# mouzzarr/go-libp2p-pubsub

Hardware: AMD Instinct MI355X
Metric: peer-heartbeat updates/sec + msg-edge deliveries/sec, 1M-peer gossipsub sim (higher is better)
Workload: dtype f64; 1 GPU; c3: 1000000 peers, random-regular k=32, one IP per peer, 16 topics, beacon-style params, 4 msg/s/topic, 10 rounds/heartbeat; peers_per_gpu=1000000, degree=32, topics=16, edge_topic_records=512000000, rounds_per_heartbeat=10

## Files before the change

### go-libp2p-pubsub_amd/csrc/deliver.hip

```cpp
#include <algorithm>
#include <cstdlib>
#include <vector>

#include "gsim_internal.h"
#include "philox.h"

namespace gsim {

#ifndef GSIM_IH_MASK
#define GSIM_IH_MASK 1
#endif
constexpr int kIhMaskSlots = 128;
__device__ __forceinline__ bool bit128(uint64_t w0, uint64_t w1, int k)
{
    return ((k < 64 ? w0 >> k : w1 >> (k - 64)) & 1ull) != 0;
}

constexpr int64_t kMaxPromTicks = 64;
constexpr int kMaxRing = 8192;

__device__ __forceinline__ bool verdict_penalises(uint8_t v)
{
    return v == GSIM_VERDICT_REJECT || v == GSIM_VERDICT_SIGNATURE;
}
// ... 1618 lines not shown
}

template <bool LAT, bool SP>
__global__ __launch_bounds__(256) void k_gossip_count(IhArgs a, uint32_t* gcount)
{
    extern __shared__ uint16_t s_act[];
    __shared__ int s_n;
    uint32_t* s_cnt = reinterpret_cast<uint32_t*>(s_act + ((a.ring + 1) & ~1));
    for (int w = threadIdx.x; w < 2 * a.ring; w += blockDim.x) s_cnt[w] = 0;
    if (threadIdx.x < 64) {
        const int lane = threadIdx.x;
        int n = 0;
        for (int m0 = 0; m0 < a.ring; m0 += 64) {
            const int m = m0 + lane;
            const bool act = m < a.ring && a.slot_last[m] >= a.lo_round;
            const uint64_t b = __ballot(act);
            if (act) s_act[n + __popcll(b & ((1ull << lane) - 1))] = (uint16_t)m;
            n += __popcll(b);
        }
        if (lane == 0) s_n = n;
    }
    __syncthreads();
    if (blockIdx.x == 0 && threadIdx.x == 0 && s_n > a.max_ihave) atomicOr(&a.nresp[3], 4u);
    const int lane = threadIdx.x & 63;
    const int64_t p0 = ((int64_t)blockIdx.x * 4 + (threadIdx.x >> 6)) * 64;
    const int nact = p0 < a.CN ? s_n : 0;
    const int64_t pc = p0 + lane, pl = pc;
    const bool vp = pc < a.CN;
    const uint64_t subp = vp ? a.sub[pl] : 0ull;
    const int64_t tick_round = a.tick * a.R;
    for (int k0 = 0; k0 < nact; k0 += kSlotBatch) {
        uint64_t cv[kSlotBatch];
#pragma unroll
        for (int b = 0; b < kSlotBatch; ++b) {
            const int k = k0 + b;
            const int64_t ci = (k < nact && vp) ? word_cell<SP>(a.cs, a.mtopic, s_act[k], p0 >> 6, lane) : -1;
            cv[b] = ci >= 0 ? a.cs.cell[ci] : kUnseen64;
        }
#pragma unroll
        for (int b = 0; b < kSlotBatch; ++b) {
            const int k = k0 + b;
            if (k >= nact) break;
            const uint32_t m = s_act[k];
            const int32_t t = (int32_t)a.mtopic[m];
            const bool hold = vp && holds_in_window(cv[b], a.g, a.lo_round, tick_round, a.minv[m] != 0,
                                                   (uint32_t)pl == a.morigin[m], LAT ? a.mlat[m] : 0u);
            const bool want = vp && cv[b] == kUnseen64 && ((subp >> t) & 1ull) && pl >= a.rlo && pl < a.rhi;
            const int nh = __popcll(__ballot(hold)), nw = __popcll(__ballot(want));
            if (lane == 0 && nh) atomicAdd(&s_cnt[m], (uint32_t)nh);
            if (lane == 0 && nw) atomicAdd(&s_cnt[a.ring + m], (uint32_t)nw);
        }
    }
    __syncthreads();
    for (int w = threadIdx.x; w < 2 * a.ring; w += blockDim.x)
        if (s_cnt[w]) atomicAdd(&gcount[w], s_cnt[w]);
}

#ifndef GSIM_COUNT_BATCH
#define GSIM_COUNT_BATCH 4
#endif
constexpr int kCountBatch = GSIM_COUNT_BATCH;
template <bool LAT>
__global__ __launch_bounds__(256) void k_gossip_count_mm(IhArgs a, const uint32_t* mctab, uint32_t* gcount)
{
    extern __shared__ uint32_t s_c[];
    __shared__ uint16_t s_slot[kMaxRing / 8];
    __shared__ int s_n;
    const int32_t t = block_topic(mctab, a.T, blockIdx.x);
    const int32_t R = a.topic_slots, m_lo = t * R;
    for (int w = threadIdx.x; w < 2 * R; w += blockDim.x) s_c[w] = 0;
    const int lane = threadIdx.x & 63, wid = threadIdx.x >> 6;
    if (threadIdx.x < 64) {
        int n = 0;
        for (int k0 = 0; k0 < R; k0 += 64) {
            const int k = k0 + lane;
            const bool act = k < R && a.slot_last[m_lo + k] >= a.lo_round;
            const uint64_t b = __ballot(act);
            if (act) s_slot[n + __popcll(b & ((1ull << lane) - 1))] = (uint16_t)k;
            n += __popcll(b);
        }
        if (lane == 0) s_n = n;
    }
    __syncthreads();
    if (blockIdx.x == 0 && threadIdx.x < 64) {
        int tot = 0;
        for (int m0 = 0; m0 < a.ring; m0 += 64)
            tot += __popcll(__ballot(m0 + lane < a.ring && a.slot_last[m0 + lane] >= a.lo_round));
        if (lane == 0 && tot > a.max_ihave) atomicOr(&a.nresp[3], 4u);
    }
    const int ns = s_n;
    const int64_t M = a.mcount[t];
    const int64_t tick_round = a.tick * a.R;
    for (int64_t j0 = (int64_t)(blockIdx.x - mctab[t]) * 1024 + wid * 64; j0 < M && ns; j0 += 256) {
        if (j0 >= (int64_t)(blockIdx.x - mctab[t] + 1) * 1024) break;
        const int64_t j = j0 + lane;
        const bool vp = j < M;
        const uint32_t p = vp ? member_peer(a, t, j) : 0u;
        const bool subp = vp && ((a.sub[p] >> t) & 1ull) && p >= a.rlo && p < a.rhi;
        uint64_t hw0 = 0, hw1 = 0, uw0 = 0, uw1 = 0;
        for (int q0 = 0; q0 < ns; q0 += kCountBatch) {
          uint64_t cb[kCountBatch];
#pragma unroll
          for (int b = 0; b < kCountBatch; ++b)
              cb[b] = (vp && q0 + b < ns) ? a.cs.cell[(int64_t)a.cs.cbase[m_lo + s_slot[q0 + b]] + j] : kUnseen64;
#pragma unroll
          for (int b = 0; b < kCountBatch; ++b) {
            const int q = q0 + b;
            if (q >= ns) break;
            const int k = s_slot[q];
            const uint32_t m = (uint32_t)(m_lo + k);
            const uint64_t c = cb[b];
            const bool hold = vp && holds_in_window(c, a.g, a.lo_round, tick_round, a.minv[m] != 0, p == a.morigin[m],
                                                    LAT ? a.mlat[m] : 0u);
            const bool want = subp && c == kUnseen64;
            const uint64_t kb = 1ull << (k & 63);
            if (hold) { if (k < 64) hw0 |= kb; else hw1 |= kb; }
            if (c == kUnseen64) { if (k < 64) uw0 |= kb; else uw1 |= kb; }
            const int nh = __popcll(__ballot(hold)), nw = __popcll(__ballot(want));
            if (lane == 0 && nh) atomicAdd(&s_c[k], (uint32_t)nh);
            if (lane == 0 && nw) atomicAdd(&s_c[R + k], (uint32_t)nw);
          }
        }
        if (a.ihm && vp) {
            uint64_t* o = a.ihm + (a.mmb[t] + j) * 4;
            o[0] = hw0; o[1] = hw1; o[2] = uw0; o[3] = uw1;
        }
    }
    __syncthreads();
    for (int w = threadIdx.x; w < 2 * R; w += blockDim.x)
        if (s_c[w]) atomicAdd(&gcount[(w < R ? 0 : a.ring - R) + m_lo + w], s_c[w]);
}

#ifndef GSIM_IH_WPE
#define GSIM_IH_WPE 4
#endif
#ifndef GSIM_IH_BATCH
#define GSIM_IH_BATCH 4
#endif
constexpr int kIhBatch = GSIM_IH_BATCH;
#ifndef GSIM_IH_HUB
#define GSIM_IH_HUB 1024
#endif
#ifndef GSIM_IH_SLICES
#define GSIM_IH_SLICES 8
#endif
constexpr uint32_t kIhHub = GSIM_IH_HUB;
constexpr int kIhSlices = GSIM_IH_SLICES;
#ifdef GSIM_DIAG_IH
__device__ unsigned long long g_ih_diag[16];
#define IH_D(...) __VA_ARGS__
#else
#define IH_D(...)
#endif
template <int W, bool LAT, bool SP, bool MM = false, int LP = 0>
__global__ __launch_bounds__(256, MM ? GSIM_IH_WPE : 1) void k_ihave(IhArgs a_, const uint32_t* gcount)
{
    const IhArgs& a = a_;
    extern __shared__ uint16_t s_act[];
    __shared__ int s_n;
    if (a.nresp[3] & 4u) return;
    const int wid = threadIdx.x >> 6;
    uint64_t* stage = reinterpret_cast<uint64_t*>(s_act + ((a.ring + 3) & ~3)) + wid * kRespStage;
    const uint32_t hw = LP == 2 ? a.hubw[blockIdx.x / kIhSlices] : 0u;
    const uint32_t bx = LP == 2 ? (hw & 0x07FFFFFFu) >> 2 : blockIdx.x;
    const int wsel = LP == 2 ? (int)(hw & 3u) : wid;
    const uint32_t slice = LP == 2 ? blockIdx.x % kIhSlices : 0u;
    const uint32_t nsl = LP == 2 ? (hw >> 27) + 1u : 1u;
    if (LP == 2 && slice >= nsl) return;
    const int32_t tb = MM ? block_topic(a.mmtab, a.T, bx) : 0;
    const int64_t jb = MM ? (int64_t)(bx - a.mmtab[tb]) * 256 : 0;
    const int m_lo = MM ? tb * a.topic_slots : 0, m_hi = MM ? m_lo + a.topic_slots : a.ring;
    if (threadIdx.x < 64) {
        const int lane = threadIdx.x;
        int n = 0;
        for (int m0 = m_lo; m0 < m_hi; m0 += 64) {
            const int m = m0 + lane;
            const bool act = m < m_hi && a.slot_last[m] >= a.lo_round && gcount[m] != 0 && gcount[a.ring + m] != 0;
            const bool push = act && (uint64_t)gcount[m] * 4u < (uint64_t)gcount[a.ring + m] * 32u;
            const uint64_t b = __ballot(act);
            if (act) s_act[n + __popcll(b & ((1ull << lane) - 1))] = (uint16_t)(m | (push ? 0x8000 : 0));
            n += __popcll(b);
        }
        if (lane == 0) s_n = n;
    }
    __syncthreads();
    const int lane = threadIdx.x & 63;
    const int64_t p0 = MM ? 0 : ((int64_t)blockIdx.x * 4 + wid) * 64;
    const int64_t jw = jb + wsel * 64;
    const int nact = (MM ? jw < a.mcount[tb] : p0 < a.CN) ? s_n : 0;
    const bool vp = MM ? jw + lane < a.mcount[tb] : p0 + lane < a.CN;
    const int64_t pl = MM ? (vp ? (int64_t)member_peer(a, tb, jw + lane) : 0) : p0 + lane;
    const int grp = lane / W, gl = lane % W;
    const uint64_t gmask = group_mask<W>(grp);
    const uint64_t subp = vp ? a.sub[pl] : 0ull;
    const uint32_t rp0 = vp ? a.row_ptr[pl] : 0u;
    const uint32_t rp1 = vp ? a.row_ptr[pl + 1] : 0u;
    const bool ign_l = vp && (a.behaviour[pl] & GSIM_BEHAVE_IGNORE_IWANT);
    const uint64_t long_lanes = W < 64 ? __ballot(rp1 - rp0 > 4u * (uint32_t)W) : 0ull;
    const uint64_t hub_lanes = LP ? __ballot(rp1 - rp0 > kIhHub) : 0ull;
    bool had_hub = false;
    uint32_t hub_max = LP == 1 && rp1 - rp0 > kIhHub ? rp1 - rp0 : 0u;
    if constexpr (LP == 1)
        for (int o = 32; o; o >>= 1) hub_max = max(hub_max, (uint32_t)__shfl_xor((int)hub_max, o, 64));
    const int64_t tick_round = a.tick * a.R;
    int nstage = 0;
    unsigned long long n_walk = 0, n_req = 0, n_resp = 0;
    auto flush_stage = [&]() {
        __builtin_amdgcn_wave_barrier();
        __builtin_amdgcn_fence(__ATOMIC_ACQ_REL, "wavefront");
        uint32_t base = 0;
        if (lane == 0 && nstage) base = atomicAdd(&a.nresp[0], (uint32_t)nstage);
        base = __shfl(base, 0, 64);
        for (int q = lane; q < nstage; q += 64) {
            if ((int64_t)base + q < a.resp_cap) a.resp[base + q] = stage[q];
            else atomicOr(&a.nresp[1], 1u);
        }
        nstage = 0;
    };
    for (int k0 = 0; !MM && k0 < nact; k0 += kSlotBatch) {
        uint64_t cv[kSlotBatch];
#pragma unroll
        for (int b = 0; b < kSlotBatch; ++b) {
            const int k = k0 + b;
            const int64_t ci = (k < nact && vp)
                                   ? (MM ? (int64_t)a.cs.cbase[s_act[k] & 0x7FFF] + jw + lane
                                         : word_cell<SP>(a.cs, a.mtopic, s_act[k] & 0x7FFF, p0 >> 6, lane))
                                   : -1;
            cv[b] = ci >= 0 ? a.cs.cell[ci] : kUnseen64;
        }
#pragma unroll
        for (int b = 0; b < kSlotBatch; ++b) {
            const IhArgs& a = kernarg0(a_);
            const int k = k0 + b;
            if (k >= nact) break;
            const uint32_t m = s_act[k] & 0x7FFF;
            const bool push = (s_act[k] & 0x8000) != 0;
            const int32_t t = (int32_t)a.mtopic[m];
            const uint32_t origin = a.morigin[m];
            const bool inv = a.minv[m] != 0;
            const bool me = vp && (push ? holds_in_window(cv[b], a.g, a.lo_round, tick_round, inv, (uint32_t)pl == origin,
                                                          LAT ? a.mlat[m] : 0u)
                                        : (cv[b] == kUnseen64 && ((subp >> t) & 1ull) && pl >= a.rlo && pl < a.rhi));
            const uint64_t mask = __ballot(me);
            if (!mask) continue;
            const int64_t cb_m = (int64_t)a.cs.cbase[m];
            auto chunk = [&](uint32_t off, uint32_t gl_, uint32_t beg, uint32_t deg, uint32_t me_id, uint32_t me_g,
                             bool ign_s, int64_t me_pl) {
                const bool v = off + gl_ < deg;
                const uint32_t e = beg + off + gl_;
                bool req = false, resp = false;
                uint32_t r = 0;
                if (push) {
                    if (v && me_pl >= 0 && a.gsel[me_pl + e]) {
                        const uint32_t p = a.col[e], re = a.rev[e];
                        const int64_t pci = a.cs.at(cb_m, t, p);
                        req = p >= a.rlo && p < a.rhi && a.gstate[re] && pci >= 0 && a.cs.cell[pci] == kUnseen64;
                        if (req) {
                            if (a.tr.ev) trace_iwant(a, p, me_id, m);
                            const uint64_t key = pair_key(a.seed, (uint32_t)a.tick, a.gid ? a.gid[p] : p, 0, P_PROMISE,
                                                          m, me_g);
                            atomicMin(reinterpret_cast<unsigned long long*>(&a.pcand[re]), (unsigned long long)key);
                            r = e;
                            resp = a.respond && a.gstate[e] && !ign_s && peertx_allows(a, m, e, me_id);
                        }
                    }
                } else {
                    if (v) {
                        const uint32_t re = a.rev[e];
                        const uint32_t i = a.col[e];
                        const uint64_t mi = smask_of(a.smask, i);
                        if (slot_has(mi, t) && a.gsel[slot_idx(mi, t, a.E, re)] && a.gstate[e]) {
                            const int64_t ici = a.cs.at(cb_m, t, i);
                            req = holds_in_window(ici >= 0 ? a.cs.cell[ici] : kUnseen64, a.g, a.lo_round, tick_round, inv,
                                                  i == origin, LAT ? a.mlat[m] : 0u);
                            if (req) {
                                if (a.tr.ev) trace_iwant(a, me_id, i, m);
                                const uint64_t key = pair_key(a.seed, (uint32_t)a.tick, me_g, 0, P_PROMISE, m,
                                                              a.gid ? a.gid[i] : i);
                                atomicMin(reinterpret_cast<unsigned long long*>(&a.pcand[e]), (unsigned long long)key);
                                r = re;
                                resp = a.respond && a.gstate[re] && !(a.behaviour[i] & GSIM_BEHAVE_IGNORE_IWANT) &&
                                       peertx_allows(a, m, re, i);
                            }
                        }
                    }
                }
                n_req += req;
                n_resp += resp;
                const uint64_t sb = __ballot(resp);
                if (sb) {
                    if (nstage + __popcll(sb) > kRespStage) flush_stage();
                    if (resp) stage[nstage + __popcll(sb & ((1ull << lane) - 1))] = (uint64_t)r | ((uint64_t)m << 32);
                    nstage += __popcll(sb);
                }
            };
            const uint64_t longm = mask & long_lanes;
            uint64_t gm = mask & ~longm & gmask;
            while (__ballot(gm != 0)) {
                int bs = -1;
                if (gm) { bs = __ffsll((long long)gm) - 1; gm &= gm - 1; }
                const int sl = bs < 0 ? lane : bs;
                const uint32_t beg = __shfl(rp0, sl, 64), end = __shfl(rp1, sl, 64);
                const bool ign_s = __shfl(ign_l, sl, 64);
                const uint32_t me_id = MM ? (uint32_t)__shfl((int)pl, sl, 64) : (uint32_t)(p0 + (bs < 0 ? 0 : bs));
                const uint32_t me_g = a.gid ? a.gid[me_id] : me_id;
                const uint64_t me_m = smask_of(a.smask, me_id);
                const int64_t me_pl = slot_has(me_m, t) ? slot_idx(me_m, t, a.E, 0) : -1;
                n_walk += (gl == 0 && bs >= 0);
                const uint32_t deg = bs >= 0 ? end - beg : 0u;
                for (uint32_t off = 0; __ballot(off < deg) != 0; off += W)
                    chunk(off, (uint32_t)gl, beg, deg, me_id, me_g, ign_s, me_pl);
            }
            for (uint64_t lm = longm; lm; lm &= lm - 1) {
                const int bs = __builtin_ctzll(lm);
                const uint32_t beg = __shfl(rp0, bs, 64), end = __shfl(rp1, bs, 64);
                const bool ign_s = __shfl(ign_l, bs, 64);
                const uint32_t me_id = MM ? (uint32_t)__shfl((int)pl, bs, 64) : (uint32_t)(p0 + bs);
                const uint32_t me_g = a.gid ? a.gid[me_id] : me_id;
                const uint64_t me_m = smask_of(a.smask, me_id);
                const int64_t me_pl = slot_has(me_m, t) ? slot_idx(me_m, t, a.E, 0) : -1;
                n_walk += (lane == 0);
                for (uint32_t off = 0; off < end - beg; off += 64)
                    chunk(off, (uint32_t)lane, beg, end - beg, me_id, me_g, ign_s, me_pl);
            }
        }
    }
    IH_D(unsigned long long d_pw = 0, d_pe = 0, d_ph = 0, d_qw = 0, d_qe = 0, d_qh = 0, d_pc = 0, d_qc = 0;)
    if constexpr (MM) {
        IH_D(const unsigned long long c_p0 = clock64();)
        const bool msk = a.ihm != nullptr;
        uint64_t ih0 = 0, ih1 = 0, iu0 = 0, iu1 = 0;
        if (msk && vp) {
            const uint64_t* o = a.ihm + (a.mmb[tb] + jw + lane) * 4;
            ih0 = o[0]; ih1 = o[1]; iu0 = o[2]; iu1 = o[3];
        }
        int64_t own_pl = -1;
        if (vp) {
            const uint64_t om = smask_of(a.smask, (uint32_t)pl);
            own_pl = slot_has(om, tb) ? slot_idx(om, tb, a.E, 0) : -1;
        }
        uint64_t pk0 = 0, pk1 = 0;
        if (msk) {
            for (int q = lane; q < nact; q += 64) {
                const uint16_t sa = s_act[q];
                if (!(sa & 0x8000)) continue;
                const int k = (int)(sa & 0x7FFF) - m_lo;
                if (k < 64) pk0 |= 1ull << k; else pk1 |= 1ull << (k - 64);
            }
            for (int o = 32; o; o >>= 1) {
                pk0 |= (uint64_t)__shfl_xor((long long)pk0, o, 64);
                pk1 |= (uint64_t)__shfl_xor((long long)pk1, o, 64);
            }
        }
        for (int k0 = 0; k0 < nact; k0 += msk ? nact : 64) {
            const int kn = nact - k0 < 64 ? nact - k0 : 64;
            uint64_t hm = 0, hm1 = 0;
            if (msk) {
                if (vp) { hm = ih0 & pk0; hm1 = ih1 & pk1; }
            } else {
                for (int q = 0; q < kn; ++q) {
                    const uint16_t sa = s_act[k0 + q];
                    if (!(sa & 0x8000)) continue;
                    const uint32_t m = sa & 0x7FFF;
                    const uint64_t c = vp ? a.cs.cell[(int64_t)a.cs.cbase[m] + jw + lane] : kUnseen64;
                    if (vp && holds_in_window(c, a.g, a.lo_round, tick_round, a.minv[m] != 0, (uint32_t)pl == a.morigin[m],
                                              LAT ? a.mlat[m] : 0u))
                        hm |= 1ull << q;
                }
            }
            const uint64_t mask = __ballot((hm | hm1) != 0);
            if (!mask) continue;
            const int32_t t = tb;
            auto ask_one = [&](bool req, uint32_t m, uint32_t p, uint32_t pg, uint32_t re, uint32_t e, uint32_t me_id,
                               uint32_t me_g, bool ign_s) {
                bool resp = false;
                if (req) {
                    if (a.tr.ev) trace_iwant(a, p, me_id, m);
                    const uint64_t key = pair_key(a.seed, (uint32_t)a.tick, pg, 0, P_PROMISE, m, me_g);
                    atomicMin(reinterpret_cast<unsigned long long*>(&a.pcand[re]), (unsigned long long)key);
                    resp = a.respond && a.gstate[e] && !ign_s && peertx_allows(a, m, e, me_id);
                }
                n_req += req;
                n_resp += resp;
                const uint64_t sb = __ballot(resp);
                if (sb) {
                    if (nstage + __popcll(sb) > kRespStage) flush_stage();
                    if (resp) stage[nstage + __popcll(sb & ((1ull << lane) - 1))] = (uint64_t)e | ((uint64_t)m << 32);
                    nstage += __popcll(sb);
                }
            };
            auto hchunk = [&](uint32_t off, uint32_t gl_, uint32_t beg, uint32_t deg, uint32_t me_id, uint32_t me_g,
                              bool ign_s, int64_t me_pl, uint64_t hmw, uint64_t hmw1) {
                const bool v = off + gl_ < deg;
                const uint32_t e = beg + off + gl_;
                uint32_t p = 0, re = 0;
                bool gs = false;
                if (v && me_pl >= 0 && a.gsel[me_pl + e]) {
                    p = a.col[e];
                    re = a.rev[e];
                    gs = p >= a.rlo && p < a.rhi && a.gstate[re];
                    IH_D(d_ph++;)
                }
                IH_D(d_pe += v;)
                const uint32_t pg = gs ? (a.gid ? a.gid[p] : p) : 0u;
                const int64_t poff = gs ? a.cs.at(0, t, p) : -1;
                if (msk) {
                    uint64_t r0 = 0, r1 = 0;
                    if (poff >= 0) {
                        const uint64_t* o = a.ihm + (a.mmb[t] + poff) * 4 + 2;
                        r0 = hmw & o[0];
                        r1 = hmw1 & o[1];
                    }
                    while (__ballot((r0 | r1) != 0)) {
                        int k = -1;
                        if (r0) { k = __builtin_ctzll(r0); r0 &= r0 - 1; }
                        else if (r1) { k = 64 + __builtin_ctzll(r1); r1 &= r1 - 1; }
                        ask_one(k >= 0, (uint32_t)(m_lo + (k < 0 ? 0 : k)), p, pg, re, e, me_id, me_g, ign_s);
                    }
                    return;
                }
                const uint64_t mine = gs ? hmw : 0ull;
                uint64_t uw = mine;
                for (int o = 32; o; o >>= 1) uw |= (uint64_t)__shfl_xor((long long)uw, o, 64);
                while (uw) {
                  int qb[kIhBatch];
                  bool ask[kIhBatch];
                  uint64_t cvb[kIhBatch];
#pragma unroll
                  for (int b = 0; b < kIhBatch; ++b) {
                      qb[b] = uw ? __builtin_ctzll(uw) : -1;
                      if (uw) uw &= uw - 1;
                      ask[b] = qb[b] >= 0 && ((mine >> qb[b]) & 1ull) && poff >= 0;
                      cvb[b] = ask[b] ? a.cs.cell[(int64_t)a.cs.cbase[s_act[k0 + qb[b]] & 0x7FFF] + poff] : 0ull;
                  }
#pragma unroll
                  for (int b = 0; b < kIhBatch; ++b) {
                    const int q = qb[b];
                    if (q < 0) break;
                    ask_one(ask[b] && cvb[b] == kUnseen64, s_act[k0 + q] & 0x7FFF, p, pg, re, e, me_id, me_g, ign_s);
                  }
                }
            };
            had_hub = had_hub || (mask & hub_lanes) != 0;
            const uint64_t longm = LP == 2 ? (mask & hub_lanes) : LP == 1 ? (mask & long_lanes & ~hub_lanes)
                                                                           : (mask & long_lanes);
            uint64_t gm = LP == 2 ? 0ull : (mask & ~long_lanes & gmask);
            while (__ballot(gm != 0)) {
                int bs = -1;
                if (gm) { bs = __ffsll((long long)gm) - 1; gm &= gm - 1; }
                const int sl = bs < 0 ? lane : bs;
                const uint32_t beg = __shfl(rp0, sl, 64), end = __shfl(rp1, sl, 64);
                const bool ign_s = __shfl(ign_l, sl, 64);
                const uint32_t me_id = (uint32_t)__shfl((int)pl, sl, 64);
                const uint64_t hmw = bs < 0 ? 0ull : (uint64_t)__shfl((long long)hm, sl, 64);
                const uint64_t hmw1 = bs < 0 ? 0ull : (uint64_t)__shfl((long long)hm1, sl, 64);
                const uint32_t me_g = a.gid ? a.gid[me_id] : me_id;
                const int64_t me_pl = (int64_t)__shfl((long long)own_pl, sl, 64);
                n_walk += (gl == 0 && bs >= 0);
                IH_D(d_pw += (gl == 0 && bs >= 0);)
                const uint32_t deg = bs >= 0 ? end - beg : 0u;
                for (uint32_t off = 0; __ballot(off < deg) != 0; off += W)
                    hchunk(off, (uint32_t)gl, beg, deg, me_id, me_g, ign_s, me_pl, hmw, hmw1);
            }
            for (uint64_t lm = longm; lm; lm &= lm - 1) {
                const int bs = __builtin_ctzll(lm);
                const uint32_t beg = __shfl(rp0, bs, 64), end = __shfl(rp1, bs, 64);
                const bool ign_s = __shfl(ign_l, bs, 64);
                const uint32_t me_id = (uint32_t)__shfl((int)pl, bs, 64);
                const uint64_t hmw = (uint64_t)__shfl((long long)hm, bs, 64);
                const uint64_t hmw1 = (uint64_t)__shfl((long long)hm1, bs, 64);
                const uint32_t me_g = a.gid ? a.gid[me_id] : me_id;
                const int64_t me_pl = (int64_t)__shfl((long long)own_pl, bs, 64);
                n_walk += (lane == 0 && slice == 0);
                IH_D(d_pw += (lane == 0 && slice == 0);)
                for (uint32_t off = slice * 64; off < end - beg; off += 64 * nsl)
                    hchunk(off, (uint32_t)lane, beg, end - beg, me_id, me_g, ign_s, me_pl, hmw, hmw1);
            }
        }
        IH_D(const unsigned long long c_p1 = clock64(); d_pc += c_p1 - c_p0;)
        const bool rcv = vp && ((subp >> tb) & 1ull) && pl >= a.rlo && pl < a.rhi;
        for (int k0 = 0; k0 < nact; k0 += 64) {
            const int kn = nact - k0 < 64 ? nact - k0 : 64;
            uint64_t wm = 0;
            for (int q = 0; q < kn; ++q) {
                const uint16_t sa = s_act[k0 + q];
                if (sa & 0x8000) continue;
                if (msk) {
                    if (rcv && bit128(iu0, iu1, (int)(sa & 0x7FFF) - m_lo)) wm |= 1ull << q;
                    continue;
                }
                const uint64_t c = rcv ? a.cs.cell[(int64_t)a.cs.cbase[sa & 0x7FFF] + jw + lane] : 0ull;
                if (rcv && c == kUnseen64) wm |= 1ull << q;
            }
            const uint64_t mask = __ballot(wm != 0);
            if (!mask) continue;
            const int32_t t = tb;
            auto pchunk = [&](uint32_t off, uint32_t gl_, uint32_t beg, uint32_t deg, uint32_t me_id, uint32_t me_g, uint64_t wmw) {
                const bool v = off + gl_ < deg;
                const uint32_t e = beg + off + gl_;
                uint32_t re = 0, i = 0;
                bool gs = false;
                if (v) {
                    re = a.rev[e];
                    i = a.col[e];
                    const uint64_t mi = smask_of(a.smask, i);
                    gs = slot_has(mi, t) && a.gsel[slot_idx(mi, t, a.E, re)] && a.gstate[e];
                }
                IH_D(d_qe += v; d_qh += gs;)
                const uint64_t mine = gs ? wmw : 0ull;
                uint64_t uw = mine;
                for (int o = 32; o; o >>= 1) uw |= (uint64_t)__shfl_xor((long long)uw, o, 64);
                const uint32_t ig = gs ? (a.gid ? a.gid[i] : i) : 0u;
                const int64_t ioff = gs ? a.cs.at(0, t, i) : -1;
                uint64_t ah0 = 0, ah1 = 0;
                if (msk && ioff >= 0) {
                    const uint64_t* o = a.ihm + (a.mmb[t] + ioff) * 4;
                    ah0 = o[0]; ah1 = o[1];
                }
                while (uw) {
                  int qb[kIhBatch];
                  uint64_t cvb[kIhBatch];
#pragma unroll
                  for (int b = 0; b < kIhBatch; ++b) {
                      qb[b] = uw ? __builtin_ctzll(uw) : -1;
                      if (uw) uw &= uw - 1;
                      const bool ask = qb[b] >= 0 && ((mine >> qb[b]) & 1ull) && ioff >= 0;
                      const uint32_t mb = ask ? s_act[k0 + qb[b]] & 0x7FFF : 0u;
                      cvb[b] = !ask ? kUnseen64 : msk ? (bit128(ah0, ah1, (int)mb - m_lo) ? 1ull : kUnseen64)
                                                      : a.cs.cell[(int64_t)a.cs.cbase[mb] + ioff];
                  }
#pragma unroll
                  for (int b = 0; b < kIhBatch; ++b) {
                    const int q = qb[b];
                    if (q < 0) break;
                    const uint32_t m = s_act[k0 + q] & 0x7FFF;
                    bool req = false, resp = false;
                    if ((mine >> q) & 1ull) {
                        req = msk ? cvb[b] != kUnseen64
                                  : holds_in_window(cvb[b], a.g, a.lo_round, tick_round,
                                                    a.minv[m] != 0, i == a.morigin[m], LAT ? a.mlat[m] : 0u);
                        if (req) {
                            if (a.tr.ev) trace_iwant(a, me_id, i, m);
                            const uint64_t key = pair_key(a.seed, (uint32_t)a.tick, me_g, 0, P_PROMISE, m, ig);
                            atomicMin(reinterpret_cast<unsigned long long*>(&a.pcand[e]), (unsigned long long)key);
                            resp = a.respond && a.gstate[re] && !(a.behaviour[i] & GSIM_BEHAVE_IGNORE_IWANT) &&
                                   peertx_allows(a, m, re, i);
                        }
                    }
                    n_req += req;
                    n_resp += resp;
                    const uint64_t sb = __ballot(resp);
                    if (sb) {
                        if (nstage + __popcll(sb) > kRespStage) flush_stage();
                        if (resp) stage[nstage + __popcll(sb & ((1ull << lane) - 1))] = (uint64_t)re | ((uint64_t)m << 32);
                        nstage += __popcll(sb);
                    }
                  }
                }
            };
            had_hub = had_hub || (mask & hub_lanes) != 0;
            const uint64_t longm = LP == 2 ? (mask & hub_lanes) : LP == 1 ? (mask & long_lanes & ~hub_lanes)
                                                                           : (mask & long_lanes);
            uint64_t gm = LP == 2 ? 0ull : (mask & ~long_lanes & gmask);
            while (__ballot(gm != 0)) {
                int bs = -1;
                if (gm) { bs = __ffsll((long long)gm) - 1; gm &= gm - 1; }
                const int sl = bs < 0 ? lane : bs;
                const uint32_t beg = __shfl(rp0, sl, 64), end = __shfl(rp1, sl, 64);
                const uint32_t me_id = (uint32_t)__shfl((int)pl, sl, 64);
                const uint64_t wmw = bs < 0 ? 0ull : (uint64_t)__shfl((long long)wm, sl, 64);
                const uint32_t me_g = a.gid ? a.gid[me_id] : me_id;
                n_walk += (gl == 0 && bs >= 0);
                IH_D(d_qw += (gl == 0 && bs >= 0);)
                const uint32_t deg = bs >= 0 ? end - beg : 0u;
                for (uint32_t off = 0; __ballot(off < deg) != 0; off += W) pchunk(off, (uint32_t)gl, beg, deg, me_id, me_g, wmw);
            }
            for (uint64_t lm = longm; lm; lm &= lm - 1) {
                const int bs = __builtin_ctzll(lm);
                const uint32_t beg = __shfl(rp0, bs, 64), end = __shfl(rp1, bs, 64);
                const uint32_t me_id = (uint32_t)__shfl((int)pl, bs, 64);
                const uint64_t wmw = (uint64_t)__shfl((long long)wm, bs, 64);
                const uint32_t me_g = a.gid ? a.gid[me_id] : me_id;
                n_walk += (lane == 0 && slice == 0);
                IH_D(d_qw += (lane == 0 && slice == 0);)
                for (uint32_t off = slice * 64; off < end - beg; off += 64 * nsl)
                    pchunk(off, (uint32_t)lane, beg, end - beg, me_id, me_g, wmw);
            }
        }
        IH_D(d_qc += clock64() - c_p1;)
        if constexpr (LP == 1) {
            if (had_hub && lane == 0) {
                const uint32_t ns = (uint32_t)kIhSlices;
                (void)hub_max;
                a.hubw[atomicAdd(a.hubn, 1u)] = (blockIdx.x * 4u + (uint32_t)wid) | ((ns - 1u) << 27);
            }
        }
    }
    flush_stage();
#ifdef GSIM_DIAG_IH
    if (MM && LP) {
        unsigned long long* dg = g_ih_diag + (LP == 2 ? 8 : 0);
        const unsigned long long v6[6] = {wave_sum_u64(d_pw), wave_sum_u64(d_pe), wave_sum_u64(d_ph),
                                          wave_sum_u64(d_qw), wave_sum_u64(d_qe), wave_sum_u64(d_qh)};
        if (lane == 0) {
            for (int q = 0; q < 6; ++q) if (v6[q]) atomicAdd(&dg[q], v6[q]);
            atomicAdd(&dg[6], d_pc);
            atomicAdd(&dg[7], d_qc);
        }
    }
#endif
    n_walk = wave_sum_u64(n_walk);
    n_req = wave_sum_u64(n_req);
    n_resp = wave_sum_u64(n_resp);
    if (lane == 0 && (n_walk | n_req)) {
        atomicAdd(&a.gstats[0], n_walk);
        atomicAdd(&a.gstats[1], n_req);
        atomicAdd(&a.gstats[2], n_resp);
    }
}

constexpr int kPairTopics = 64;

template <bool LAT>
__global__ __launch_bounds__(256) void k_ihave_pairs(IhArgs a)
{
    extern __shared__ uint16_t s_act[];
    __shared__ int s_n;
    if (!(a.nresp[3] & 4u)) return;
    const int wid = threadIdx.x >> 6, lane = threadIdx.x & 63;
    uint64_t* base = reinterpret_cast<uint64_t*>(s_act + ((a.ring + 3) & ~3));
    uint64_t* stage = base + wid * kRespStage;
    uint64_t* s_tau = base + 4 * kRespStage + wid * kPairTopics;
    uint32_t* s_cnt = reinterpret_cast<uint32_t*>(base + 4 * kRespStage + 4 * kPairTopics) + wid * kPairTopics;
    if (threadIdx.x < 64) {
        int n = 0;
        for (int m0 = 0; m0 < a.ring; m0 += 64) {
            const int m = m0 + lane;
            const bool act = m < a.ring && a.slot_last[m] >= a.lo_round;
            const uint64_t b = __ballot(act);
            if (act) s_act[n + __popcll(b & ((1ull << lane) - 1))] = (uint16_t)m;
            n += __popcll(b);
        }
        if (lane == 0) s_n = n;
    }
    __syncthreads();
    const int ns = s_n;
    const uint32_t L = (uint32_t)a.max_ihave;
    const int64_t tick_round = a.tick * a.R;
    int nstage = 0;
    unsigned long long n_walk = 0, n_req = 0, n_resp = 0;
    auto flush_stage = [&]() {
        __builtin_amdgcn_wave_barrier();
        __builtin_amdgcn_fence(__ATOMIC_ACQ_REL, "wavefront");
        uint32_t b0 = 0;
        if (lane == 0 && nstage) b0 = atomicAdd(&a.nresp[0], (uint32_t)nstage);
        b0 = __shfl(b0, 0, 64);
        for (int q = lane; q < nstage; q += 64) {
            if ((int64_t)b0 + q < a.resp_cap) a.resp[b0 + q] = stage[q];
            else atomicOr(&a.nresp[1], 1u);
        }
        nstage = 0;
    };
    auto lds_sync = [&]() {
        __builtin_amdgcn_fence(__ATOMIC_RELEASE, "wavefront");
        __builtin_amdgcn_wave_barrier();
        __builtin_amdgcn_fence(__ATOMIC_ACQUIRE, "wavefront");
    };
    auto kth_key = [&](auto sel) -> uint64_t {
        uint64_t lo = 0, hi = ~0ull;
        while (lo < hi) {
            const uint64_t mid = lo + ((hi - lo) >> 1);
            uint32_t c = 0;
            for (int k0 = 0; k0 < ns; k0 += 64) {
                const int k = k0 + lane;
                uint64_t key = 0;
                c += (uint32_t)__popcll(__ballot(k < ns && sel(k, key) && key <= mid));
            }
            if (c >= L) hi = mid; else lo = mid + 1;
        }
        return lo;
    };
    for (int64_t pc = (int64_t)blockIdx.x * 4 + wid; pc < a.CN; pc += (int64_t)gridDim.x * 4) {
        const uint32_t p = (uint32_t)pc;
        if (p < a.rlo || p >= a.rhi) continue;
        const uint64_t subp = a.sub[p];
        const uint32_t beg = a.row_ptr[p], end = a.row_ptr[p + 1];
        const uint32_t p_g = a.gid ? a.gid[p] : p;
        for (uint32_t e = beg; e < end; ++e) {
            if (!a.gstate[e]) continue;
            const uint32_t re = a.rev[e], i = a.col[e];
            const uint64_t mi = smask_of(a.smask, i);
            const bool tb = lane < a.T && ((subp >> lane) & 1ull) && slot_has(mi, lane) &&
                            a.gsel[slot_idx(mi, lane, a.E, re)];
            const uint64_t tmask = __ballot(tb);
            if (!tmask) continue;
            n_walk += (lane == 0);
            const uint32_t i_g = a.gid ? a.gid[i] : i;
            const uint32_t origin_ign = a.behaviour[i] & GSIM_BEHAVE_IGNORE_IWANT;
            auto holds = [&](uint32_t m) {
                return holds_in_window(a.cs.get(m, (int32_t)a.mtopic[m], i), a.g, a.lo_round, tick_round, a.minv[m] != 0,
                                       i == a.morigin[m], LAT ? a.mlat[m] : 0u);
            };
            s_cnt[lane] = 0;
            lds_sync();
            for (int k0 = 0; k0 < ns; k0 += 64) {
                const int k = k0 + lane;
                if (k < ns) {
                    const uint32_t m = s_act[k];
                    const int t = (int)a.mtopic[m];
                    if (((tmask >> t) & 1ull) && holds(m)) atomicAdd(&s_cnt[t], 1u);
                }
            }
            lds_sync();
            const uint64_t omask = __ballot(s_cnt[lane] > L) & tmask;
            for (uint64_t om = omask; om; om &= om - 1) {
                const int t = __ffsll((long long)om) - 1;
                const uint64_t tau = kth_key([&](int k, uint64_t& key) {
                    const uint32_t m = s_act[k];
                    if ((int)a.mtopic[m] != t || !holds(m)) return false;
                    key = pair_key(a.seed, (uint32_t)a.tick, i_g, (uint32_t)t, P_IHAVE_TRUNC, m, p_g);
                    return true;
                });
                if (lane == 0) s_tau[t] = tau;
            }
            lds_sync();
            auto wanted = [&](uint32_t m) {
                const int t = (int)a.mtopic[m];
                if (!((tmask >> t) & 1ull) || a.cs.get(m, t, p) != kUnseen64 || !holds(m)) return false;
                return s_cnt[t] <= L ||
                       pair_key(a.seed, (uint32_t)a.tick, i_g, (uint32_t)t, P_IHAVE_TRUNC, m, p_g) <= s_tau[t];
            };
            uint32_t nw = 0;
            for (int k0 = 0; k0 < ns; k0 += 64) {
                const int k = k0 + lane;
                nw += (uint32_t)__popcll(__ballot(k < ns && wanted(s_act[k])));
            }
            if (nw == 0) continue;
            uint64_t tau_w = ~0ull;
            if (nw > L)
                tau_w = kth_key([&](int k, uint64_t& key) {
                    const uint32_t m = s_act[k];
                    if (!wanted(m)) return false;
                    key = pair_key(a.seed, (uint32_t)a.tick, p_g, 0, P_IWANT, m, i_g);
                    return true;
                });
            uint64_t pmin = ~0ull;
            for (int k0 = 0; k0 < ns; k0 += 64) {
                const int k = k0 + lane;
                const uint32_t m = k < ns ? s_act[k] : 0u;
                const bool ask = k < ns && wanted(m) &&
                                 (nw <= L || pair_key(a.seed, (uint32_t)a.tick, p_g, 0, P_IWANT, m, i_g) <= tau_w);
                bool resp = false;
                if (ask) {
// ... 783 lines not shown
int deliver_promise_check(gsim_handle* h, int64_t now)
{
    Deliver* d = h->dl;
    if (!d) return GSIM_OK;
    for (int q = 0; q < d->prom_ticks; ++q) {
        const int64_t made = d->prom_made[(size_t)q];
        if (made < 0) continue;
        const int64_t expire = round_time_host(d, made * d->cfg.rounds) + h->gp.iwant_followup_time_ns;
        if (!(expire < now)) continue;
        hipLaunchKernelGGL(k_promise_check, dim3(std::min<int64_t>((h->e + 255) / 256, 16384)), dim3(256), 0,
                           h->stream, d->d_prom + (size_t)q * (size_t)h->e, deliver_cells(d),
                           (const uint32_t*)d->d_mtopic, (const uint32_t*)h->d_owner, (const uint32_t*)h->d_rev,
                           h->d_pen, h->e, d->d_gstats);
        d->prom_made[(size_t)q] = -1;
        int rc = hip_check(h, hipGetLastError(), "k_promise_check");
        if (rc) return rc;
    }
    return GSIM_OK;
}

int deliver_heartbeat_begin(gsim_handle* h, uint64_t tick)
{
    Deliver* d = h->dl;
    if (!d) return GSIM_OK;
    d->ihave_tick = (int64_t)tick;
    return GSIM_OK;
}

namespace gsim {
struct IhaveStage {
    IhArgs a{};
    size_t lds, lds_c;
    int grid;
};
}

static bool ihave_prepare(gsim_handle* h, int64_t g, IhaveStage* st, int* rc)
{
    *rc = GSIM_OK;
    Deliver* d = h->dl;
    const int64_t tick = g / d->cfg.rounds;
    if (d->ihave_tick != tick) return false;
    d->ihave_tick = -1;
    if (h->gp.max_ihave_messages < 1 || h->gp.max_ihave_length < 1) return false;
    IhArgs& a = st->a;
    a = IhArgs{};
    a.N = h->n; a.E = h->e; a.T = h->t; a.ring = d->cfg.ring; a.R = d->cfg.rounds;
    a.g = g; a.tick = tick;
    a.lo_round = (int32_t)std::max<int64_t>((tick - h->gp.history_gossip) * d->cfg.rounds, 0);
    a.serve_lo = (int32_t)std::max<int64_t>((tick - h->gp.history_length + 1) * d->cfg.rounds, 0);
    a.row_ptr = h->d_row_ptr; a.col = h->d_col; a.rev = h->d_rev; a.sub = h->d_sub; a.smask = h->d_smask;
    a.mtopic = d->d_mtopic; a.morigin = d->d_morigin; a.minv = d->d_minv;
    a.mlat = d->lat_on ? d->d_mlat : nullptr;
    a.cs = deliver_cells(d); a.slot_last = d->d_slot_last;
    a.gsel = d->d_gsel; a.gstate = d->d_gstate; a.behaviour = d->d_behaviour;
    a.pcand = d->d_pcand; a.prom = d->d_prom; a.P = d->prom_ticks;
    a.prom_idx = (int32_t)(tick % d->prom_ticks);
    if (d->prom_made[(size_t)a.prom_idx] >= 0) {
        h->err = "IWANT promise ring index still pending (refresh_scores must run every heartbeat)";
        *rc = GSIM_ESTATE;
        return false;
    }
    d->prom_made[(size_t)a.prom_idx] = tick;
    a.resp = d->d_resp; a.nresp = d->d_nresp; a.resp_cap = d->resp_cap; a.gstats = d->d_gstats;
    a.respond = h->gp.gossip_retransmission >= 1;
    a.seed = h->x ? gsim_get_seed(h) : 0;
    a.CN = h->n;
    a.rlo = (uint32_t)h->olo();
    a.rhi = (uint32_t)h->ohi();
    if (ShardCtx* sh = h->sh) {
        a.sharded = 1;
        a.gid = sh->d_gid;
    }
    a.max_ihave = h->gp.max_ihave_length;
    a.tr = h->trace;
    a.t0 = d->cfg.t0_ns; a.hb = d->cfg.heartbeat_ns; a.roff = d->d_roff;
    a.peertx = d->d_peertx; a.ptx_w = d->ptx_w;
    a.retrans = h->gp.gossip_retransmission;
    if (mm_gossip(h)) {
        a.mlist = d->d_mlist; a.mloff = d->d_mloff; a.mcount = d->d_mcount; a.mmtab = d->d_mmtab;
        a.topic_slots = (int32_t)d->cfg.topic_slots;
        a.ihm = d->d_ihm; a.mmb = d->d_mmb;
        const int64_t need = 4 * (int64_t)(d->mmtab.empty() ? 0 : d->mmtab.back());
        if (need > d->hubw_cap) {
            if (d->d_hubw) { (void)hipFree(d->d_hubw); d->d_hubw = nullptr; d->hubw_cap = 0; }
            if (hipMalloc((void**)&d->d_hubw, sizeof(uint32_t) * (size_t)(need + 1)) == hipSuccess) d->hubw_cap = need;
        }
        if (d->d_hubw && need > 0) {
            a.hubw = d->d_hubw;
            a.hubn = d->d_hubw + d->hubw_cap;
        }
    }
    st->lds = (((size_t)d->cfg.ring + 3) & ~(size_t)3) * sizeof(uint16_t) + 4 * kRespStage * sizeof(uint64_t);
    st->lds_c = (((size_t)d->cfg.ring + 1) & ~(size_t)1) * sizeof(uint16_t) + 2 * (size_t)d->cfg.ring * 4;
    st->grid = grid_peers(a.CN);
    hipError_t e = hipMemsetAsync(d->d_nresp, 0, 2 * sizeof(uint32_t), h->stream);
    if (e == hipSuccess) e = hipMemsetAsync(d->d_nresp + 3, 0, sizeof(uint32_t), h->stream);
    if (e == hipSuccess) e = hipMemsetAsync(d->d_gcount, 0, 2 * (size_t)d->cfg.ring * 4, h->stream);
    if (e != hipSuccess) { *rc = hip_check(h, e, "gossip reset"); return false; }
    return true;
}

static int ihave_count(gsim_handle* h, IhaveStage* st)
{
    ProfScope ps(h, GSIM_K_GOSSIP);
    Deliver* d = h->dl;
    if (st->a.mmtab) {
        const uint32_t grid = d->mctab.back();
        const size_t lds = 2 * (size_t)d->cfg.topic_slots * 4;
        if (grid && st->a.mlat)
            hipLaunchKernelGGL(k_gossip_count_mm<true>, dim3(grid), dim3(256), lds, h->stream, st->a,
                               (const uint32_t*)d->d_mctab, d->d_gcount);
        else if (grid)
            hipLaunchKernelGGL(k_gossip_count_mm<false>, dim3(grid), dim3(256), lds, h->stream, st->a,
                               (const uint32_t*)d->d_mctab, d->d_gcount);
    } else if (st->a.mlat)
        hipLaunchKernelGGL((k_gossip_count<true, true>), dim3(st->grid), dim3(256), st->lds_c, h->stream, st->a, h->dl->d_gcount);
    else if (sparse_layout(h))
        hipLaunchKernelGGL((k_gossip_count<false, true>), dim3(st->grid), dim3(256), st->lds_c, h->stream, st->a, h->dl->d_gcount);
    else
        hipLaunchKernelGGL((k_gossip_count<false, false>), dim3(st->grid), dim3(256), st->lds_c, h->stream, st->a, h->dl->d_gcount);
    return hip_check(h, hipGetLastError(), "k_gossip_count");
}

template <int W>
static void launch_ihave_w(gsim_handle* h, IhaveStage* st, const IhArgs& a)
{
    if (a.mmtab) {
        const uint32_t grid = h->dl->mmtab.back();
        if (!grid) return;
        const uint32_t* gc = h->dl->d_gcount;
        if (a.hubw && W < 64) {
            uint32_t n = 0;
            hipError_t e = hipMemsetAsync(a.hubn, 0, sizeof(uint32_t), h->stream);
            if (e != hipSuccess) return;
            if (a.mlat)
                hipLaunchKernelGGL((k_ihave<W, true, true, true, 1>), dim3(grid), dim3(256), st->lds, h->stream, a, gc);
            else
                hipLaunchKernelGGL((k_ihave<W, false, true, true, 1>), dim3(grid), dim3(256), st->lds, h->stream, a, gc);
            e = hipMemcpyAsync(&n, a.hubn, sizeof(uint32_t), hipMemcpyDeviceToHost, h->stream);
            if (e == hipSuccess) e = hipStreamSynchronize(h->stream);
            if (e != hipSuccess || n == 0) return;
            const uint32_t g2 = n * (uint32_t)kIhSlices;
            if (a.mlat)
                hipLaunchKernelGGL((k_ihave<W, true, true, true, 2>), dim3(g2), dim3(64), st->lds, h->stream, a, gc);
            else
                hipLaunchKernelGGL((k_ihave<W, false, true, true, 2>), dim3(g2), dim3(64), st->lds, h->stream, a, gc);
            return;
        }
        if (a.mlat)
            hipLaunchKernelGGL((k_ihave<W, true, true, true>), dim3(grid), dim3(256), st->lds, h->stream, a, gc);
        else
            hipLaunchKernelGGL((k_ihave<W, false, true, true>), dim3(grid), dim3(256), st->lds, h->stream, a, gc);
    } else if (a.mlat)
        hipLaunchKernelGGL((k_ihave<W, true, true>), dim3(st->grid), dim3(256), st->lds, h->stream, a, (const uint32_t*)h->dl->d_gcount);
    else if (sparse_layout(h))
        hipLaunchKernelGGL((k_ihave<W, false, true>), dim3(st->grid), dim3(256), st->lds, h->stream, a, (const uint32_t*)h->dl->d_gcount);
    else
        hipLaunchKernelGGL((k_ihave<W, false, false>), dim3(st->grid), dim3(256), st->lds, h->stream, a, (const uint32_t*)h->dl->d_gcount);
}

static int ihave_walk(gsim_handle* h, IhaveStage* st)
{
    Deliver* d = h->dl;
    IhArgs& a = st->a;
    ProfScope ps(h, GSIM_K_GOSSIP);
    int w = h->ihave_w;
    if (w == 0) {
        const bool short_mean = h->e <= 24 * (int64_t)h->n;
        w = (h->max_degree <= 16 || (h->max_degree > 32 && short_mean)) ? 16 : h->max_degree <= 32 ? 32 : 64;
    }
    if (w == 8)
        launch_ihave_w<8>(h, st, a);
    else if (w == 16)
        launch_ihave_w<16>(h, st, a);
    else if (w == 32)
        launch_ihave_w<32>(h, st, a);
    else
        launch_ihave_w<64>(h, st, a);
    if (d->cfg.ring > h->gp.max_ihave_length) {
        const size_t lds = (((size_t)d->cfg.ring + 3) & ~(size_t)3) * sizeof(uint16_t) +
                           4 * (kRespStage + kPairTopics) * sizeof(uint64_t) + 4 * kPairTopics * sizeof(uint32_t);
        const int grid = (int)std::min<int64_t>((a.CN + 3) / 4, 4096);
        if (a.mlat) hipLaunchKernelGGL(k_ihave_pairs<true>, dim3(grid), dim3(256), lds, h->stream, a);
        else hipLaunchKernelGGL(k_ihave_pairs<false>, dim3(grid), dim3(256), lds, h->stream, a);
    }
    hipLaunchKernelGGL(k_promise_insert, dim3(std::min<int64_t>((h->e + 255) / 256, 16384)), dim3(256), 0, h->stream,
                       d->d_pcand, d->d_prom, d->prom_ticks, a.prom_idx, h->e);
    d->resp_round = a.g + 2;
    d->resp_marked = false;
    return hip_check(h, hipGetLastError(), "k_ihave");
}

static int launch_ihave(gsim_handle* h, int64_t g)
{
    IhaveStage st;
    int rc = GSIM_OK;
    if (!ihave_prepare(h, g, &st, &rc)) return rc;
    rc = ihave_count(h, &st);
    if (!rc) rc = ihave_walk(h, &st);
    return rc;
}

int deliver_flush(gsim_handle* h)
{
    Deliver* d = h->dl;
    if (!d || d->pending < 0) return GSIM_OK;
    ProfScope ps(h, GSIM_K_COMMIT);
    RoundArgs a = make_round_args(h, d->pending);
    a.flist_commit = a.flist != nullptr;
    d->flist_round = a.flist ? d->pending + 1 : -1;
    const int gp = grid_peers((int64_t)a.rhi - ((int64_t)a.rlo & ~63ll));
    const dim3 grid(sparse_layout(h) ? std::min(gp, 8192) : gp);
    const bool split = gp < 4096 && h->sh && !a.mlat && !a.gt.act && !sparse_layout(h);
    if (a.clist)
        hipLaunchKernelGGL(k_commit_list<true>, dim3(64, kClSub), dim3(256), 0, h->stream, a);
    if (a.mlat)
        hipLaunchKernelGGL((k_commit<true, true>), grid, dim3(256), (size_t)d->cfg.ring * sizeof(uint16_t), h->stream, a);
    else if (a.gt.act && sparse_layout(h))
        hipLaunchKernelGGL((k_commit<false, true, true>), grid, dim3(256), (size_t)d->cfg.ring * sizeof(uint16_t), h->stream, a);
    else if (a.gt.act)
        hipLaunchKernelGGL((k_commit<false, false, true>), grid, dim3(256), (size_t)d->cfg.ring * sizeof(uint16_t), h->stream, a);
    else if (sparse_layout(h))
        hipLaunchKernelGGL((k_commit<false, true>), grid, dim3(256), (size_t)d->cfg.ring * sizeof(uint16_t), h->stream, a);
    else if (split)
        hipLaunchKernelGGL((k_commit<false, false, false, true>), dim3(gp, GSIM_SPLIT_GROUPS), dim3(256),
                           (size_t)d->cfg.ring * sizeof(uint16_t),
                           h->stream, a);
    else
        hipLaunchKernelGGL((k_commit<false, false>), grid, dim3(256), (size_t)d->cfg.ring * sizeof(uint16_t), h->stream, a);
    const int64_t committed = d->pending;
    d->pending = -1;
    hipError_t e = hipGetLastError();
    if (e == hipSuccess && a.clist) e = hipMemsetAsync(d->d_clist_n, 0, (kClSub + 1) * kClStride * sizeof(uint32_t), h->stream);
    const int rc = hip_check(h, e, "k_commit");
    return rc ? rc : gater_fold(h, committed, a.now);
}

static int vq_check(gsim_handle* h)
{
    Deliver* d = h->dl;
    if (!d->lat_on) return GSIM_OK;
    uint32_t ov = 0;
    hipError_t e = hipMemcpyAsync(&ov, d->d_vqn + kVqOver, sizeof(ov), hipMemcpyDeviceToHost, h->stream);
    if (e == hipSuccess) e = hipStreamSynchronize(h->stream);
    if (e != hipSuccess) return hip_check(h, e, "validation queue flag");
    if (ov) { h->err = "copies pending validation overflowed their queue (raise gsim_msg_config.max_arrivals)"; return GSIM_ERANGE; }
    return GSIM_OK;
}

int deliver_check_errors(gsim_handle* h)
{
    Deliver* d = h->dl;
    if (!d) return GSIM_OK;
    if (int rc = vq_check(h)) return rc;
    uint32_t err[4] = {0, 0, 0, 0};
    hipError_t e = hipMemcpyAsync(err, d->d_nresp, sizeof(err), hipMemcpyDeviceToHost, h->stream);
    if (e == hipSuccess) e = hipStreamSynchronize(h->stream);
    if (e != hipSuccess) return hip_check(h, e, "delivery error flags");
    if (err[1]) { h->err = "IWANT responses overflowed their queue (raise gsim_msg_config.max_arrivals)"; return GSIM_ERANGE; }
    if (err[2]) {
        h->err = "a ring slot was republished while its message could still be gossiped or promised (raise ring)";
        return GSIM_ESTATE;
    }
    return GSIM_OK;
}

bool deliver_trace_view(gsim_handle* h, TraceView* v)
{
    Deliver* d = h->dl;
    if (!d) return false;
    v->cells = deliver_cells(d); v->mtopic = d->d_mtopic; v->minv = d->d_minv; v->mid = d->d_mid;
    v->ring = d->cfg.ring; v->rounds = d->cfg.rounds;
    v->mlat = d->lat_on ? d->d_mlat : nullptr;
    v->t0 = d->cfg.t0_ns; v->hb = d->cfg.heartbeat_ns; v->roff = d->d_roff;
    return true;
}

bool deliver_report_view(gsim_handle* h, ReportView* v)
{
    Deliver* d = h->dl;
    if (!d) return false;
    v->cells = deliver_cells(d); v->ncells = (int64_t)d->n_cells;
    v->mtopic = d->d_mtopic; v->morigin = d->d_morigin; v->minv = d->d_minv; v->mlat = d->d_mlat; v->mid = d->d_mid;
    v->mpub = d->d_mpub; v->slot_last = d->d_slot_last;
    v->ring = d->cfg.ring; v->T = h->t; v->n = h->n;
    v->rlo = (uint32_t)h->olo(); v->rhi = (uint32_t)h->ohi();
    v->sub = h->d_sub;
    return true;
}

int64_t deliver_next_round(gsim_handle* h)
{
    const Deliver* d = h->dl;
    return d && d->next_round > 0 ? d->next_round : 0;
}

int64_t deliver_last_round_time(gsim_handle* h)
{
    const Deliver* d = h->dl;
    if (!d || d->next_round <= 0) return INT64_MAX;
    return round_time_host(d, d->next_round - 1);
}

int deliver_read_seen(gsim_handle* h, void* dst)
{
    Deliver* d = h->dl;
    int rc = deliver_flush(h);
    if (rc) return rc;
    const size_t n = (size_t)d->cfg.ring * (size_t)h->n;
    hipError_t e = hipSuccess;
    if (!d->d_seen32) e = hipMalloc((void**)&d->d_seen32, std::max<size_t>(n * 4, 4));
// ... 1459 lines not shown
```

Measured before the change: 22.94 million peer-heartbeat updates/sec.

## Flatten push-side IHAVE edge walk into wave-wide work queue via LDS

For push-mode IHAVE slots in the non-MM kernel, each lane first builds a 64-bit bitmask of its gossip-selected edges by reading eight selection bytes at a time. The wave then prefix-sums the per-lane counts and packs (lane, edge) pairs into a small per-wave LDS table, so all 64 lanes process selected edges together instead of walking each peer's row in groups. The aim is to skip unselected edges and improve lane use when few edges per row are selected. In exchange it needs extra LDS, adds shuffles and wave barriers, and also moves the dense launch-bounds occupancy hint behind a new macro.

```diff
diff --git a/go-libp2p-pubsub_amd/csrc/deliver.hip b/go-libp2p-pubsub_amd/csrc/deliver.hip
--- a/go-libp2p-pubsub_amd/csrc/deliver.hip
+++ b/go-libp2p-pubsub_amd/csrc/deliver.hip
@@ -1794,8 +1794,41 @@
 #else
 #define IH_D(...)
 #endif
+#ifndef GSIM_IH_FLAT
+#define GSIM_IH_FLAT 1
+#endif
+#ifndef GSIM_IH_WPE_DENSE
+#define GSIM_IH_WPE_DENSE 1
+#endif
+constexpr bool kIhFlat = GSIM_IH_FLAT != 0;
+constexpr uint32_t kIhFlatRow = 64;
+constexpr int kIhFlatTab = 256;
+constexpr size_t kIhFlatLds = kIhFlat ? 4 * kIhFlatTab * sizeof(uint16_t) : 0;
+
+__device__ __forceinline__ uint64_t nz_bytes8(const uint8_t* s)
+{
+    uint64_t w;
+    __builtin_memcpy(&w, s, 8);
+    const uint64_t k7 = 0x7F7F7F7F7F7F7F7Full;
+    const uint64_t nz = ((((w & k7) + k7) | w) & ~k7) >> 7;
+    return (nz * 0x0102040810204080ull) >> 56;
+}
+__device__ __forceinline__ uint64_t row_sel_mask(const uint8_t* s, uint32_t deg)
+{
+    uint64_t m = 0;
+#pragma unroll
+    for (uint32_t j = 0; j < kIhFlatRow / 8; ++j)
+        if (8 * j + 8 <= deg) m |= nz_bytes8(s + 8 * j) << (8 * j);
+    if (deg >= 8) {
+        if (deg & 7u) m |= nz_bytes8(s + deg - 8) << (deg - 8);
+    } else {
+        for (uint32_t q = 0; q < deg; ++q) m |= (uint64_t)(s[q] != 0) << q;
+    }
+    return m;
+}
+
 template <int W, bool LAT, bool SP, bool MM = false, int LP = 0>
-__global__ __launch_bounds__(256, MM ? GSIM_IH_WPE : 1) void k_ihave(IhArgs a_, const uint32_t* gcount)
+__global__ __launch_bounds__(256, MM ? GSIM_IH_WPE : GSIM_IH_WPE_DENSE) void k_ihave(IhArgs a_, const uint32_t* gcount)
 {
     const IhArgs& a = a_;
     extern __shared__ uint16_t s_act[];
@@ -1803,6 +1836,7 @@
     if (a.nresp[3] & 4u) return;
     const int wid = threadIdx.x >> 6;
     uint64_t* stage = reinterpret_cast<uint64_t*>(s_act + ((a.ring + 3) & ~3)) + wid * kRespStage;
+    uint16_t* ftab = reinterpret_cast<uint16_t*>(stage + (4 - wid) * kRespStage) + wid * kIhFlatTab;
     const uint32_t hw = LP == 2 ? a.hubw[blockIdx.x / kIhSlices] : 0u;
     const uint32_t bx = LP == 2 ? (hw & 0x07FFFFFFu) >> 2 : blockIdx.x;
     const int wsel = LP == 2 ? (int)(hw & 3u) : wid;
@@ -1859,6 +1893,8 @@
         }
         nstage = 0;
     };
+    IH_D(unsigned long long d_pw = 0, d_pe = 0, d_ph = 0, d_qw = 0, d_qe = 0, d_qh = 0, d_pc = 0, d_qc = 0;)
+    const uint32_t own_g = !MM && kIhFlat && a.gid && vp ? a.gid[pl] : (uint32_t)pl;
     for (int k0 = 0; !MM && k0 < nact; k0 += kSlotBatch) {
         uint64_t cv[kSlotBatch];
 #pragma unroll
@@ -1886,14 +1922,27 @@
             const uint64_t mask = __ballot(me);
             if (!mask) continue;
             const int64_t cb_m = (int64_t)a.cs.cbase[m];
+            IH_D(const unsigned long long c_s0 = clock64();)
+            auto emit = [&](bool req, bool resp, uint32_t r) {
+                n_req += req;
+                n_resp += resp;
+                const uint64_t sb = __ballot(resp);
+                if (sb) {
+                    if (nstage + __popcll(sb) > kRespStage) flush_stage();
+                    if (resp) stage[nstage + __popcll(sb & ((1ull << lane) - 1))] = (uint64_t)r | ((uint64_t)m << 32);
+                    nstage += __popcll(sb);
+                }
+            };
             auto chunk = [&](uint32_t off, uint32_t gl_, uint32_t beg, uint32_t deg, uint32_t me_id, uint32_t me_g,
                              bool ign_s, int64_t me_pl) {
                 const bool v = off + gl_ < deg;
                 const uint32_t e = beg + off + gl_;
                 bool req = false, resp = false;
                 uint32_t r = 0;
+                IH_D(if (push) d_pe += v; else d_qe += v;)
                 if (push) {
                     if (v && me_pl >= 0 && a.gsel[me_pl + e]) {
+                        IH_D(d_ph++;)
                         const uint32_t p = a.col[e], re = a.rev[e];
                         const int64_t pci = a.cs.at(cb_m, t, p);
                         req = p >= a.rlo && p < a.rhi && a.gstate[re] && pci >= 0 && a.cs.cell[pci] == kUnseen64;
@@ -1912,6 +1961,7 @@
                         const uint32_t i = a.col[e];
                         const uint64_t mi = smask_of(a.smask, i);
                         if (slot_has(mi, t) && a.gsel[slot_idx(mi, t, a.E, re)] && a.gstate[e]) {
+                            IH_D(d_qh++;)
                             const int64_t ici = a.cs.at(cb_m, t, i);
                             req = holds_in_window(ici >= 0 ? a.cs.cell[ici] : kUnseen64, a.g, a.lo_round, tick_round, inv,
                                                   i == origin, LAT ? a.mlat[m] : 0u);
@@ -1927,17 +1977,73 @@
                         }
                     }
                 }
-                n_req += req;
-                n_resp += resp;
-                const uint64_t sb = __ballot(resp);
-                if (sb) {
-                    if (nstage + __popcll(sb) > kRespStage) flush_stage();
-                    if (resp) stage[nstage + __popcll(sb & ((1ull << lane) - 1))] = (uint64_t)r | ((uint64_t)m << 32);
-                    nstage += __popcll(sb);
+                emit(req, resp, r);
+            };
+            uint64_t flat = 0;
+            if (kIhFlat && push) {
+                const uint32_t dl = rp1 - rp0;
+                const bool fl = me && dl <= kIhFlatRow;
+                flat = __ballot(fl);
+                if (flat) {
+                    uint64_t tm = 0;
+                    if (fl && dl) {
+                        const uint64_t om = smask_of(a.smask, (uint32_t)pl);
+                        if (slot_has(om, t)) tm = row_sel_mask(a.gsel + slot_idx(om, t, a.E, rp0), dl);
+                    }
+                    n_walk += fl;
+                    IH_D(d_pw += fl; d_pe += fl ? dl : 0u; d_ph += (unsigned)__popcll(tm);)
+                    const uint32_t cnt = (uint32_t)__popcll(tm);
+                    uint32_t inc = cnt;
+#pragma unroll
+                    for (int o = 1; o < 64; o <<= 1) {
+                        const uint32_t up = (uint32_t)__shfl_up((int)inc, o, 64);
+                        if (lane >= o) inc += up;
+                    }
+                    const uint32_t total = (uint32_t)__shfl((int)inc, 63, 64);
+                    uint32_t ni = inc - cnt;
+                    for (uint32_t w0 = 0; w0 < total; w0 += kIhFlatTab) {
+                        const uint32_t wn = total - w0 < (uint32_t)kIhFlatTab ? total - w0 : (uint32_t)kIhFlatTab;
+                        while (tm && ni < w0 + wn) {
+                            ftab[ni - w0] = (uint16_t)((lane << 8) | __builtin_ctzll(tm));
+                            tm &= tm - 1;
+                            ++ni;
+                        }
+                        __builtin_amdgcn_wave_barrier();
+                        __builtin_amdgcn_fence(__ATOMIC_ACQ_REL, "wavefront");
+                        for (uint32_t q0 = 0; q0 < wn; q0 += 64) {
+                            const bool v = q0 + lane < wn;
+                            const uint32_t pr = v ? ftab[q0 + lane] : (uint32_t)lane << 8;
+                            const int hl = (int)(pr >> 8);
+                            const uint32_t e = (uint32_t)__shfl((int)rp0, hl, 64) + (pr & 0xFFu);
+                            const bool ign_s = __shfl((int)ign_l, hl, 64) != 0;
+                            const uint32_t me_g = (uint32_t)__shfl((int)own_g, hl, 64);
+                            const uint32_t me_id = (uint32_t)(p0 + hl);
+                            bool req = false, resp = false;
+                            if (v) {
+                                const uint32_t p = a.col[e], re = a.rev[e];
+                                const uint8_t ge = a.gstate[e];
+                                const bool own = p >= a.rlo && p < a.rhi;
+                                const int64_t pci = own ? a.cs.at(cb_m, t, p) : -1;
+                                const uint8_t gr = own ? a.gstate[re] : (uint8_t)0;
+                                const uint64_t pc = pci >= 0 ? a.cs.cell[pci] : 0ull;
+                                req = gr && pci >= 0 && pc == kUnseen64;
+                                if (req) {
+                                    if (a.tr.ev) trace_iwant(a, p, me_id, m);
+                                    const uint64_t key = pair_key(a.seed, (uint32_t)a.tick, a.gid ? a.gid[p] : p, 0,
+                                                                  P_PROMISE, m, me_g);
+                                    atomicMin(reinterpret_cast<unsigned long long*>(&a.pcand[re]), (unsigned long long)key);
+                                    resp = a.respond && ge && !ign_s && peertx_allows(a, m, e, me_id);
+                                }
+                            }
+                            emit(req, resp, e);
+                        }
+                        __builtin_amdgcn_wave_barrier();
+                        __builtin_amdgcn_fence(__ATOMIC_ACQ_REL, "wavefront");
+                    }
                 }
-            };
-            const uint64_t longm = mask & long_lanes;
-            uint64_t gm = mask & ~longm & gmask;
+            }
+            const uint64_t longm = mask & long_lanes & ~flat;
+            uint64_t gm = mask & ~longm & ~flat & gmask;
             while (__ballot(gm != 0)) {
                 int bs = -1;
                 if (gm) { bs = __ffsll((long long)gm) - 1; gm &= gm - 1; }
@@ -1949,6 +2055,7 @@
                 const uint64_t me_m = smask_of(a.smask, me_id);
                 const int64_t me_pl = slot_has(me_m, t) ? slot_idx(me_m, t, a.E, 0) : -1;
                 n_walk += (gl == 0 && bs >= 0);
+                IH_D(if (push) d_pw += (gl == 0 && bs >= 0); else d_qw += (gl == 0 && bs >= 0);)
                 const uint32_t deg = bs >= 0 ? end - beg : 0u;
                 for (uint32_t off = 0; __ballot(off < deg) != 0; off += W)
                     chunk(off, (uint32_t)gl, beg, deg, me_id, me_g, ign_s, me_pl);
@@ -1962,12 +2069,13 @@
                 const uint64_t me_m = smask_of(a.smask, me_id);
                 const int64_t me_pl = slot_has(me_m, t) ? slot_idx(me_m, t, a.E, 0) : -1;
                 n_walk += (lane == 0);
+                IH_D(if (push) d_pw += (lane == 0); else d_qw += (lane == 0);)
                 for (uint32_t off = 0; off < end - beg; off += 64)
                     chunk(off, (uint32_t)lane, beg, end - beg, me_id, me_g, ign_s, me_pl);
             }
-        }
-    }
-    IH_D(unsigned long long d_pw = 0, d_pe = 0, d_ph = 0, d_qw = 0, d_qe = 0, d_qh = 0, d_pc = 0, d_qc = 0;)
+            IH_D(if (push) d_pc += clock64() - c_s0; else d_qc += clock64() - c_s0;)
+        }
+    }
     if constexpr (MM) {
         IH_D(const unsigned long long c_p0 = clock64();)
         const bool msk = a.ihm != nullptr;
@@ -2240,7 +2348,7 @@
     }
     flush_stage();
 #ifdef GSIM_DIAG_IH
-    if (MM && LP) {
+    if (!MM || LP) {
         unsigned long long* dg = g_ih_diag + (LP == 2 ? 8 : 0);
         const unsigned long long v6[6] = {wave_sum_u64(d_pw), wave_sum_u64(d_pe), wave_sum_u64(d_ph),
                                           wave_sum_u64(d_qw), wave_sum_u64(d_qe), wave_sum_u64(d_qh)};
@@ -3330,12 +3438,15 @@
             hipLaunchKernelGGL((k_ihave<W, true, true, true>), dim3(grid), dim3(256), st->lds, h->stream, a, gc);
         else
             hipLaunchKernelGGL((k_ihave<W, false, true, true>), dim3(grid), dim3(256), st->lds, h->stream, a, gc);
-    } else if (a.mlat)
-        hipLaunchKernelGGL((k_ihave<W, true, true>), dim3(st->grid), dim3(256), st->lds, h->stream, a, (const uint32_t*)h->dl->d_gcount);
+        return;
+    }
+    const size_t lds = st->lds + kIhFlatLds;
+    if (a.mlat)
+        hipLaunchKernelGGL((k_ihave<W, true, true>), dim3(st->grid), dim3(256), lds, h->stream, a, (const uint32_t*)h->dl->d_gcount);
     else if (sparse_layout(h))
-        hipLaunchKernelGGL((k_ihave<W, false, true>), dim3(st->grid), dim3(256), st->lds, h->stream, a, (const uint32_t*)h->dl->d_gcount);
+        hipLaunchKernelGGL((k_ihave<W, false, true>), dim3(st->grid), dim3(256), lds, h->stream, a, (const uint32_t*)h->dl->d_gcount);
     else
-        hipLaunchKernelGGL((k_ihave<W, false, false>), dim3(st->grid), dim3(256), st->lds, h->stream, a, (const uint32_t*)h->dl->d_gcount);
+        hipLaunchKernelGGL((k_ihave<W, false, false>), dim3(st->grid), dim3(256), lds, h->stream, a, (const uint32_t*)h->dl->d_gcount);
 }
 
 static int ihave_walk(gsim_handle* h, IhaveStage* st)
```

Result: faster. 23.17 million peer-heartbeat updates/sec (median of 6 runs) (+1.0%).
